# biotite-dev/springcraft

Measured on AMD Instinct MI355X. Metric: ANM modes/sec (Hessian build + full eigensolve), N=2000 C-alpha, higher is better.
Workload: dtype f64; 1 GPU; C3: N=2000 C-alpha ANM, HinsenForceField (no cutoff), full 6000x6000 eigensolve, all modes + vectors; parallelism=independent structures sharded over GPUs, no data-path collective

## Files before the change

### springcraft_amd/csrc/sb2st.hip

```cpp
#include <algorithm>

#include "twostage_internal.h"

namespace {

__global__ void k_xcd_probe(unsigned* mask) {
  unsigned id;
  asm volatile("s_getreg_b32 %0, hwreg(HW_REG_XCC_ID)" : "=s"(id));
  if (threadIdx.x == 0) atomicOr(mask, 1u << (id & 15u));
}
int probe_xcd_count(sc_ctx* ctx, hipStream_t st) {
  SC_TRY(sc_reserve_dc_aux(ctx, 256));
  unsigned* d_mask = reinterpret_cast<unsigned*>(ctx->dc_aux);
  SC_HIP(ctx, hipMemsetAsync(d_mask, 0, sizeof(unsigned), st));
  const int cus = ctx->num_cus > 0 ? ctx->num_cus : 256;
  hipLaunchKernelGGL(k_xcd_probe, dim3((unsigned)(8 * cus)), dim3(64), 0, st, d_mask);
  SC_HIP(ctx, hipGetLastError());
  unsigned h_mask = 0;
  SC_HIP(ctx, hipMemcpyAsync(&h_mask, d_mask, sizeof(unsigned), hipMemcpyDeviceToHost, st));
  SC_HIP(ctx, hipStreamSynchronize(st));
  int count = 0, top = 0;
  for (int b = 0; b < 16; ++b)
    if (h_mask >> b & 1u) { ++count; top = b + 1; }
  ctx->nxcd = (count >= 1 && count == top) ? std::min(count, 8) : 1;
// ... 257 lines not shown
#ifdef CHASE_STAMPS
__device__ unsigned long long g_chase_stamps[16];
#define CHASE_STAMP_DECL unsigned long long cs_prev = 0, cs_n = 0, cs_sum[12] = {0, 0, 0, 0, 0, 0, 0, 0, 0, 0, 0, 0};
#define CHASE_STAMP(i)                                                                 \
  {                                                                                    \
    unsigned long long t_;                                                             \
    asm volatile("s_memtime %0\n\ts_waitcnt lgkmcnt(0)" : "=s"(t_)::"memory");        \
    if ((i) != 0) cs_sum[i] += t_ - cs_prev;                                           \
    cs_prev = t_;                                                                      \
  }
#define CHASE_STAMP_WRITE                                                                          \
  if ((threadIdx.x & 63) == 0) {                                                                   \
    for (int i_ = 1; i_ < 12; ++i_) atomicAdd(&g_chase_stamps[i_], cs_sum[i_]);                    \
    atomicAdd(&g_chase_stamps[15], cs_n);                                                          \
  }
#else
#define CHASE_STAMP_DECL
#define CHASE_STAMP(i)
#define CHASE_STAMP_WRITE
#endif
template <int SPREAD>
__global__ __launch_bounds__(256, 2) void k_bulge_chase(double* __restrict__ sb_all, SbLayout SL, int batch, int W, int nxcd,
                                                     int* __restrict__ progress, int* __restrict__ next_sweep,
                                                     int* __restrict__ ctl, int give_up_after, v4i* __restrict__ early) {
  constexpr int LD = kB + 1;
  __shared__ double E[kB * LD];
  double* D = E;
  __shared__ double vbuf[2][kB], u[kB], red[4 * kB];
  __shared__ double s_tau, s_beta, s_beta_in;
  __shared__ int s_go, s_claim, s_mode;

  const int n = SL.n;
  const int tid = threadIdx.x;
  const int i = tid & 63, q = tid >> 6;
  __shared__ int s_xcd, s_slot;
  if (tid == 0) {
    unsigned id;
    asm volatile("s_getreg_b32 %0, hwreg(HW_REG_XCC_ID)" : "=s"(id));
    s_xcd = (int)(id & 7u) % nxcd;
    s_slot = atomicAdd(ctl + 2 + s_xcd, 1);
  }
  __syncthreads();
  const int xcd = s_xcd, slot = s_slot;
  const int mpx = xcd < batch ? (batch - xcd + nxcd - 1) / nxcd : 0;
  if (mpx == 0 || slot >= mpx * W) return;
  const int K0 = chase_len(n, 0);
  int tasks_left = give_up_after;

  CHASE_STAMP_DECL
  int cur = slot % mpx, exhausted = 0;
  while (exhausted < mpx) {
    const int b = xcd + nxcd * cur;
    int* prog = progress + (size_t)b * n;
    if (tid == 0) s_claim = atomicAdd(next_sweep + b, 1);
    __syncthreads();
    const int s = __builtin_amdgcn_readfirstlane(s_claim);
    __syncthreads();
    if (s > n - 3) {
      ++exhausted;
      cur = cur + 1 < mpx ? cur + 1 : 0;
      continue;
    }
    exhausted = 0;
    double* sb = sb_all + (size_t)b * SL.slab;
    double* ab = sb + SL.ab;
    {
      const int len = chase_len(n, s);
      const int S = s / kG, cc = s - S * kG;
      const size_t dia0 = (size_t)S * K0 - (size_t)S * (S - 1) / 2;
      const int len_prev = s > 0 ? chase_len(n, s - 1) : 0;
      double tau_p = 0.0;
      for (int k = 0; k < len; ++k) {
        double* vp = vbuf[(k + 1) & 1];
        double* vn = vbuf[k & 1];
        const bool early_task = early != nullptr && s > 0 && k + 1 < len_prev;
        CHASE_STAMP(0)
        if (tid == 0) {
          const int need = s > 0 ? min(k + (early_task ? 1 : 2), len_prev) : 0;
          const int stop0 = __hip_atomic_load(ctl, __ATOMIC_RELAXED, __HIP_MEMORY_SCOPE_AGENT);
          int have = s > 0 ? __hip_atomic_load(prog + s - 1, __ATOMIC_RELAXED, __HIP_MEMORY_SCOPE_AGENT) : 0;
          int go = stop0 ? 0 : 1;
          int mode = 0;
          double beta_in = 0.0;
          const v4i* rec = early_task ? early + ((size_t)b * n + s - 1) * kEarlyRing + ((k + 1) & (kEarlyRing - 1)) : nullptr;
          long spins = 0;
          while (go) {
            if (have >= need) {
              if (!early_task) break;
              if (have >= k + 2) { mode = 2; break; }
              const v4i r = ld16_l2(rec);
              if (r.z == k + 2) {
                mode = 1;
                beta_in = __longlong_as_double((long long)(((unsigned long long)(unsigned)r.y << 32) | (unsigned)r.x));
                break;
              }
            }
            ++spins;
            if (spins > (1L << 21) ||
                ((spins & 15) == 0 && __hip_atomic_load(ctl, __ATOMIC_RELAXED, __HIP_MEMORY_SCOPE_AGENT))) {
              if (!__hip_atomic_load(ctl, __ATOMIC_RELAXED, __HIP_MEMORY_SCOPE_AGENT)) {
                ctl[10] = b; ctl[11] = s; ctl[12] = k;
              }
              __hip_atomic_store(ctl, 1, __ATOMIC_RELAXED, __HIP_MEMORY_SCOPE_AGENT);
              go = 0;
              break;
            }
            __builtin_amdgcn_s_sleep(1);
            have = __hip_atomic_load(prog + s - 1, __ATOMIC_RELAXED, __HIP_MEMORY_SCOPE_AGENT);
          }
          s_go = go;
          s_mode = mode;
          s_beta_in = beta_in;
        }
        __syncthreads();
        if (!s_go) return;
        CHASE_STAMP(1)
        const int mode = s_mode;
#define CHASE_SECOND_WAIT()                                                                                       \
        if (mode == 1) {                                                                                          \
          if (tid == 0) {                                                                                         \
            int go = 1;                                                                                           \
            long spins = 0;                                                                                       \
            while (__hip_atomic_load(prog + s - 1, __ATOMIC_RELAXED, __HIP_MEMORY_SCOPE_AGENT) < k + 2) {         \
              ++spins;                                                                                            \
              if (spins > (1L << 21) ||                                                                           \
                  ((spins & 15) == 0 && __hip_atomic_load(ctl, __ATOMIC_RELAXED, __HIP_MEMORY_SCOPE_AGENT))) {    \
                if (!__hip_atomic_load(ctl, __ATOMIC_RELAXED, __HIP_MEMORY_SCOPE_AGENT)) {                        \
                  ctl[10] = b; ctl[11] = s; ctl[12] = k;                                                          \
                }                                                                                                 \
                __hip_atomic_store(ctl, 1, __ATOMIC_RELAXED, __HIP_MEMORY_SCOPE_AGENT);                           \
                go = 0;                                                                                           \
                break;                                                                                            \
              }                                                                                                   \
              __builtin_amdgcn_s_sleep(1);                                                                        \
            }                                                                                                     \
            s_go = go;                                                                                            \
          }                                                                                                       \
          __syncthreads();                                                                                        \
          if (!s_go) return;                                                                                      \
        }

        const int r0 = s + 1 + k * kB;
        const int L = min(kB, n - r0);
        const size_t dia = dia0 + k;
        double* vd = sb + SL.vd + dia * kDiaSize + (size_t)cc * kG + cc;
        gdptr colbase_k = wave_uniform(ab + (size_t)r0 * kLdab);
        double d16[16];
#pragma unroll
        for (int c = 0; c < 16; ++c) {
          const int jc = min(q * 16 + c, L - 1);
          const int ic = min(max(i, jc), L - 1);
          d16[c] = ld_l2(colbase_k + (unsigned)((ic - jc) + jc * kLdab));
        }
        if (k > 0) {
          gdptr ebase_k = wave_uniform(ab + (size_t)(r0 - kB) * kLdab);
          double t16[16];
          {
            const int ic = min(i, L - 1);
#pragma unroll
            for (int c = 0; c < 16; ++c) {
              const int jj = q * 16 + c;
              t16[c] = ld_l2(ebase_k + (unsigned)((kB + ic - jj) + jj * kLdab));
            }
#pragma unroll
            for (int c = 0; c < 16; ++c) t16[c] = i < L ? t16[c] : 0.0;
            if (mode == 1 && i == kB - 1) {
              const double bin = s_beta_in;
#pragma unroll
              for (int c = 0; c < 16; ++c) t16[c] = q * 16 + c == kB - 1 ? bin : 0.0;
            }
          }
          {
            double a = 0.0;
#pragma unroll
            for (int c = 0; c < 16; ++c) a += t16[c] * vp[q * 16 + c];
            red[q * kB + i] = a;
          }
          lds_barrier();
          CHASE_STAMP(2)
          {
            const double ui = tau_p * ((red[i] + red[kB + i]) + (red[2 * kB + i] + red[3 * kB + i]));
#pragma unroll
            for (int c = 0; c < 16; ++c) {
              t16[c] -= ui * vp[q * 16 + c];
              E[i * LD + q * 16 + c] = t16[c];
            }
          }
          if (q == 0) {
            const double x = t16[0];
            const double t2 = wave_sum((i >= 1 && i < L) ? x * x : 0.0);
            const HH h = householder(__shfl(x, 0), t2);
            vn[i] = i == 0 ? 1.0 : (i < L ? x * h.scale : 0.0);
            if (i == 0) {
              s_tau = h.tau; s_beta = h.beta;
              if (early) {
                const unsigned long long bb = (unsigned long long)__double_as_longlong(h.beta);
                if (SPREAD) st16_sc1(early + ((size_t)b * n + s) * kEarlyRing + (k & (kEarlyRing - 1)), v4i{(int)(unsigned)bb, (int)(unsigned)(bb >> 32), k + 1, 0});
                else st16(early + ((size_t)b * n + s) * kEarlyRing + (k & (kEarlyRing - 1)), v4i{(int)(unsigned)bb, (int)(unsigned)(bb >> 32), k + 1, 0});
              }
            }
          }
          lds_barrier();
          CHASE_STAMP(3)
          {
            double a = 0.0;
#pragma unroll
            for (int ii = q * 16; ii < q * 16 + 16; ++ii) a += E[ii * LD + i] * vn[ii];
            red[q * kB + i] = a;
          }
          lds_barrier();
          if (tid < kB) u[tid] = s_tau * ((red[tid] + red[kB + tid]) + (red[2 * kB + tid] + red[3 * kB + tid]));
          lds_barrier();
          CHASE_STAMP(4)
          CHASE_SECOND_WAIT()
          CHASE_STAMP(5)
#pragma unroll
          for (int c = 0; c < 16; ++c) {
            const int jj = q * 16 + c;
            double e = t16[c] - vn[i] * u[jj];
            if (jj == 0) e = i == 0 ? s_beta : 0.0;
            if (i < L) st_band<SPREAD>(ebase_k + (unsigned)((kB + i - jj) + jj * kLdab), e);
          }
        } else {
          gdptr col_s = wave_uniform(ab + (size_t)s * kLdab);
          if (tid < 64) {
            const double xr = ld_l2(col_s + (unsigned)(1 + min(tid, L - 1)));
            double x = tid < L ? xr : 0.0;
            if (mode == 1 && tid == kB - 1) x = s_beta_in;
            const double t2 = wave_sum(tid >= 1 ? x * x : 0.0);
            const HH h = householder(__shfl(x, 0), t2);
            vn[tid] = tid == 0 ? 1.0 : x * h.scale;
            if (tid == 0) { s_tau = h.tau; s_beta = h.beta; }
          }
          lds_barrier();
          CHASE_STAMP(4)
          CHASE_SECOND_WAIT()
          CHASE_STAMP(5)
          if (tid < L) st_band<SPREAD>(col_s + (unsigned)(1 + tid), tid == 0 ? s_beta : 0.0);
        }
#undef CHASE_SECOND_WAIT
        if (mode == 1 && i == kB - 1) {
#pragma unroll
          for (int c = 0; c < 16; ++c) {
            const int jc = q * 16 + c;
            d16[c] = ld_l2(colbase_k + (unsigned)((kB - 1 - jc) + jc * kLdab));
          }
        }
#pragma unroll
        for (int c = 0; c < 16; ++c) {
          const int jj = q * 16 + c;
          if (i >= jj) {
            const double x = (i < L) ? d16[c] : 0.0;
            D[i * LD + jj] = x;
            D[jj * LD + i] = x;
          }
        }
        lds_barrier();
        CHASE_STAMP(6)
        {
          double a = 0.0;
#pragma unroll
          for (int jj = q * 16; jj < q * 16 + 16; ++jj) a += D[i * LD + jj] * vn[jj];
          red[q * kB + i] = a;
        }
        lds_barrier();
        CHASE_STAMP(7)
        const double tau_now = s_tau;
        if (tid < 64) {
          const double pp = tau_now * ((red[tid] + red[kB + tid]) + (red[2 * kB + tid] + red[3 * kB + tid]));
          const double dot = wave_sum(pp * vn[tid]);
          u[tid] = pp - 0.5 * tau_now * dot * vn[tid];
        }
        lds_barrier();
        CHASE_STAMP(8)
        for (int jj = q * 16; jj < q * 16 + 16; ++jj)
          if (i >= jj && i < L)
            st_band<SPREAD>(colbase_k + (unsigned)((i - jj) + jj * kLdab), D[i * LD + jj] - vn[i] * u[jj] - u[i] * vn[jj]);
        if (tid < L) vd[(size_t)tid * kG] = vn[tid];
        if (tid == 0) sb[SL.tau2 + dia * kG + cc] = tau_now;
        tau_p = tau_now;
        CHASE_STAMP(9)
        asm volatile("s_waitcnt vmcnt(0)" ::: "memory");
        __syncthreads();
        CHASE_STAMP(10)
        if (tid == 0) {
          __hip_atomic_store(prog + s, k + 1, __ATOMIC_RELAXED, __HIP_MEMORY_SCOPE_AGENT);
          if (k + 1 == len) atomicAdd(ctl + 16 + xcd, 1);
          if (give_up_after > 0 && --tasks_left == 0) {
            ctl[1] = give_up_after;
            __hip_atomic_store(ctl, 1, __ATOMIC_RELAXED, __HIP_MEMORY_SCOPE_AGENT);
          }
        }
        CHASE_STAMP(11)
#ifdef CHASE_STAMPS
        ++cs_n;
#endif
      }
    }
  }
  CHASE_STAMP_WRITE
}

constexpr int kSlotE = kB * (kB + 1);
constexpr int kSlotD = 17 * 128;
constexpr int kSlot = kSlotE + kSlotD;
constexpr int kTeamLds = 2 * kB + kB + 4 * kB + 8;
constexpr size_t kPairLdsBytes = sizeof(double) * (3 * kSlot + 2 * kTeamLds);

#ifdef PAIR_STAMPS
__device__ unsigned long long g_pair_stamps[48];
__shared__ unsigned long long s_pair_stamps[48];
#define PAIR_STAMP(var) unsigned long long var; asm volatile("s_memtime %0\n\ts_waitcnt lgkmcnt(0)" : "=s"(var)::"memory");
#define PAIR_ACC(slot, a, b) if (tid == 0) s_pair_stamps[slot] += (b) - (a);
#define PAIR_ACC_B(slot, a, b) if (tid == 256) s_pair_stamps[16 + (slot)] += (b) - (a);
#define PAIR_FLUSH(first)                                                                         \
  for (int i_ = 0; i_ < 16; ++i_)                                                                 \
    if (s_pair_stamps[(first) + i_]) atomicAdd(&g_pair_stamps[(first) + i_], s_pair_stamps[(first) + i_]);
#else
#define PAIR_STAMP(var)
#define PAIR_ACC(slot, a, b)
#define PAIR_ACC_B(slot, a, b)
#define PAIR_FLUSH(first)
#endif

typedef double __attribute__((address_space(3)))* ldptr;
struct PairStepArgs {
  double* ab;
  double* vd;
  double* tau2;
  ldptr slots;
  ldptr vbuf, u, red, sc;
  int* prog;
  int s, k;
  size_t dia;
  int cc;
  int tid;
};

template <int TEAM>
__device__ __forceinline__ void pair_step_full(const PairStepArgs& P, double& tau_p, int& pend_k) {
  const int tid = P.tid, tt = tid & 255, i = tid & 63;
  const int q = (tid >> 6) & 3;
  const int k = P.k, s = P.s;
  const int r0 = s + 1 + k * kB;
  ldptr vp = P.vbuf + ((k + 1) & 1) * kB;
  ldptr vn = P.vbuf + (k & 1) * kB;
  ldptr Eimg = P.slots + (k % 3) * kSlot;
  ldptr Dimg = Eimg + kSlotE;
  ldptr red = P.red;
  ldptr u = P.u;
  gdptr colbase_k = wave_uniform(P.ab + (size_t)r0 * kLdab);
  gdptr ebase_k = wave_uniform(P.ab + (size_t)(r0 - kB) * kLdab);
  const unsigned o_e = (unsigned)(kB + i + q * 16 * (kLdab - 1));
  const unsigned o_d = (unsigned)(i + q * 16 * (kLdab - 1));
  double d16[16], t16[16], vr[16];
  PAIR_STAMP(f0)
  if (TEAM == 0) {
#pragma unroll
    for (int c = 0; c < 16; ++c) t16[c] = ld_l2(ebase_k + (o_e + (unsigned)(c * (kLdab - 1))));
  } else {
    const ldptr En = P.slots + ((k + 1) % 3) * kSlot;
    const int i1 = min(i + 1, kB - 1);
    const ldptr rowD = i < kB - 1 ? Dimg + i1 * (i1 + 1) / 2 : En;
    const ldptr rowE = Eimg + i1 * (kB + 1) + 1;
#pragma unroll
    for (int c = 0; c < 16; ++c) d16[c] = rowD[q * 16 + c + 1];
#pragma unroll
    for (int c = 0; c < 16; ++c) t16[c] = i < kB - 1 ? rowE[q * 16 + c] : 0.0;
    if (q == 3) {
      const double dcol = Dimg[i1 * (i1 + 1) / 2];
      t16[15] = i < kB - 1 ? dcol : En[0];
      if (i == kB - 1) d16[15] = En[kSlotE];
    }
    PAIR_STAMP(g1)
    asm volatile("s_waitcnt vmcnt(0)" ::: "memory");
    PAIR_STAMP(g2)
    PAIR_ACC_B(10, f0, g1) PAIR_ACC_B(11, g1, g2)
  }
#pragma unroll
  for (int c = 0; c < 16; ++c) vr[c] = vp[q * 16 + c];
  PAIR_STAMP(fa)
  lds_barrier();
  PAIR_STAMP(f1)
  PAIR_ACC(12, f0, fa)
  if (TEAM == 1) {
    if (tt == 0 && pend_k >= 0) __hip_atomic_store(P.prog + s, pend_k + 1, __ATOMIC_RELAXED, __HIP_MEMORY_SCOPE_AGENT);
    pend_k = k;
  } else {
#pragma unroll
    for (int c = 0; c < 16; ++c) d16[c] = ld_l2(colbase_k + (o_d + (unsigned)(c * (kLdab - 1))));
  }
  {
    double a = 0.0;
#pragma unroll
    for (int c = 0; c < 16; ++c) a += t16[c] * vr[c];
    red[q * kB + i] = a;
  }
  lds_barrier();
  {
    const double ui = tau_p * ((red[i] + red[kB + i]) + (red[2 * kB + i] + red[3 * kB + i]));
    ldptr erow = Eimg + i * (kB + 1) + q * 16;
#pragma unroll
    for (int c = 0; c < 16; ++c) {
      t16[c] -= ui * vr[c];
      erow[c] = t16[c];
    }
    if (q == 0) {
      const double x = t16[0];
      const double t2 = wave_sum(i >= 1 ? x * x : 0.0);
      const HH h = householder(__shfl(x, 0), t2);
      vn[i] = i == 0 ? 1.0 : x * h.scale;
      if (i == 0) { P.sc[0] = h.tau; P.sc[1] = h.beta; }
    }
  }
  lds_barrier();
  PAIR_STAMP(f3)
#pragma unroll
  for (int c = 0; c < 16; ++c) vr[c] = vn[q * 16 + c];
  {
    double a = 0.0;
    const ldptr ecol = Eimg + q * 16 * (kB + 1) + i;
#pragma unroll
    for (int c = 0; c < 16; ++c) a += ecol[c * (kB + 1)] * vr[c];
    red[q * kB + i] = a;
  }
  lds_barrier();
  if (tt < kB) u[tt] = P.sc[0] * ((red[tt] + red[kB + tt]) + (red[2 * kB + tt] + red[3 * kB + tt]));
  {
    ldptr rowp = Dimg + i * (i + 1) / 2 + q * 16;
#pragma unroll
    for (int c = 0; c < 16; ++c) {
      d16[c] = q * 16 + c <= i ? d16[c] : 0.0;
      if (q * 16 + c <= i) rowp[c] = d16[c];
    }
  }
  lds_barrier();
  PAIR_STAMP(f5)
  {
    const double vi = vn[i];
#pragma unroll
    for (int c = 0; c < 16; ++c) t16[c] -= vi * u[q * 16 + c];
    if (q == 0) t16[0] = i == 0 ? P.sc[1] : 0.0;
    if (TEAM == 0) {
      ldptr erow = Eimg + i * (kB + 1) + q * 16;
#pragma unroll
      for (int c = 0; c < 16; ++c) erow[c] = t16[c];
      if (q == 0 && i >= 1) ebase_k[(unsigned)(kB + i)] = 0.0;
    } else {
#pragma unroll
      for (int c = 0; c < 16; ++c) ebase_k[o_e + (unsigned)(c * (kLdab - 1))] = t16[c];
    }
    double a = 0.0;
#pragma unroll
    for (int c = 0; c < 16; ++c) {
      const int ii = q * 16 + c;
      const double dcolv = Dimg[ii * (ii + 1) / 2 + min(i, ii)];
      a += (d16[c] + (ii > i ? dcolv : 0.0)) * vr[c];
    }
    red[q * kB + i] = a;
  }
  lds_barrier();
  PAIR_STAMP(f6)
  const double tau_f = P.sc[0];
  if (tt < kB) {
    const double pp = tau_f * ((red[tt] + red[kB + tt]) + (red[2 * kB + tt] + red[3 * kB + tt]));
    const double dot = wave_sum(pp * vn[tt]);
    u[tt] = pp - 0.5 * tau_f * dot * vn[tt];
  }
  lds_barrier();
  PAIR_STAMP(f7)
  {
    const double vi = vn[i], wi = u[i];
    if (TEAM == 0) {
      ldptr rowp = Dimg + i * (i + 1) / 2 + q * 16;
#pragma unroll
      for (int c = 0; c < 16; ++c)
        if (q * 16 + c <= i) rowp[c] = d16[c] - vi * u[q * 16 + c] - wi * vr[c];
    } else {
#pragma unroll
      for (int c = 0; c < 16; ++c)
        if (q * 16 + c <= i) colbase_k[o_d + (unsigned)(c * (kLdab - 1))] = d16[c] - vi * u[q * 16 + c] - wi * vr[c];
    }
    double* vd = P.vd + P.dia * kDiaSize + (size_t)P.cc * kG + P.cc;
    if (tt < kB) vd[(size_t)tt * kG] = vn[tt];
    if (tt == 0) P.tau2[P.dia * kG + P.cc] = tau_f;
    tau_p = tau_f;
  }
#ifdef PAIR_STAMPS
  {
    PAIR_STAMP(f8)
    PAIR_ACC(1, f0, f1) PAIR_ACC(2, f1, f3) PAIR_ACC(3, f3, f5) PAIR_ACC(4, f5, f6) PAIR_ACC(5, f6, f7) PAIR_ACC(6, f7, f8)
    PAIR_ACC_B(1, f0, f1) PAIR_ACC_B(2, f1, f3) PAIR_ACC_B(3, f3, f5) PAIR_ACC_B(4, f5, f6) PAIR_ACC_B(5, f6, f7)
    PAIR_ACC_B(13, f7, f8)
  }
#endif
}

struct PairGenArgs {
  double* ab;
  double* vd;
  double* tau2;
  ldptr slots;
  ldptr vbuf, u, red, sc;
  int* prog;
  int* sweeps_done;
  int n, s, k, my_len, team, to_lds;
  size_t dia0;
  int cc, tid;
};
struct PairCarry {
  double tau_p;
  int pend_k;
};

__device__ __noinline__ PairCarry pair_step_general(const PairGenArgs P, double tau_p, int pend_k) {
  double* const ab = P.ab;
  const ldptr slots = P.slots, vbuf = P.vbuf, u = P.u, red = P.red, sc = P.sc;
  int* const prog = P.prog;
  const int n = P.n, s = P.s, k = P.k, my_len = P.my_len, team = P.team, cc = P.cc, tid = P.tid;
  const bool to_lds = P.to_lds != 0;
  const size_t dia0 = P.dia0;
  const int tt = tid & 255, i = tid & 63, q = (tid >> 6) & 3;
  const bool active = k >= 0 && k < my_len;
  const bool first = k == 0;
  const bool eph = active && !first;
  const int kk = active ? k : 0;
  const int r0 = s + 1 + kk * kB;
  const int L = active ? min(kB, n - r0) : 0;
  ldptr vp = vbuf + ((kk + 1) & 1) * kB;
  ldptr vn = vbuf + (kk & 1) * kB;
  ldptr Eimg = slots + (kk % 3) * kSlot;
  ldptr Dimg = Eimg + kSlotE;
  const size_t dia = dia0 + kk;
  gdptr colbase_k = wave_uniform(ab + (size_t)r0 * kLdab);
  gdptr ebase_k = wave_uniform(ab + (size_t)(r0 - (first ? 0 : kB)) * kLdab);

  double d16[16], t16[16];
  double xcol = 0.0;
#pragma unroll
  for (int c = 0; c < 16; ++c) { d16[c] = 0.0; t16[c] = 0.0; }
  if (active && team == 0) {
    if (!first) {
      const int ic = min(i, L - 1);
#pragma unroll
      for (int c = 0; c < 16; ++c) {
        const int jj = q * 16 + c;
        t16[c] = ld_l2(ebase_k + (unsigned)((kB + ic - jj) + jj * kLdab));
      }
    } else if (q == 0) {
      gdptr col_s = wave_uniform(ab + (size_t)s * kLdab);
      xcol = ld_l2(col_s + (unsigned)(1 + min(i, L - 1)));
    }
#pragma unroll
    for (int c = 0; c < 16; ++c) {
      const int jc = min(q * 16 + c, L - 1);
      const int ic = min(max(i, jc), L - 1);
      d16[c] = ld_l2(colbase_k + (unsigned)((ic - jc) + jc * kLdab));
    }
  } else if (active) {
    const ldptr En = slots + ((kk + 1) % 3) * kSlot;
    const int i1 = min(i + 1, kB - 1);
    const ldptr rowD = i < kB - 1 ? Dimg + i1 * (i1 + 1) / 2 : En;
    const ldptr rowE = Eimg + i1 * (kB + 1) + 1;
#pragma unroll
    for (int c = 0; c < 16; ++c) d16[c] = rowD[q * 16 + c + 1];
    if (!first) {
#pragma unroll
      for (int c = 0; c < 16; ++c) t16[c] = i < kB - 1 ? rowE[q * 16 + c] : 0.0;
    }
    if (q == 3) {
      const double dcol = Dimg[i1 * (i1 + 1) / 2];
      if (!first) t16[15] = i < kB - 1 ? dcol : En[0];
      if (i == kB - 1) d16[15] = En[kSlotE];
    }
    if (first && q == 0) xcol = i < kB - 1 ? Dimg[i1 * (i1 + 1) / 2] : En[0];
  }
#pragma unroll
  for (int c = 0; c < 16; ++c) t16[c] = i < L ? t16[c] : 0.0;
  xcol = i < L ? xcol : 0.0;
  if (!to_lds || !active) asm volatile("s_waitcnt vmcnt(0)" ::: "memory");
  lds_barrier();
  if (tt == 0 && pend_k >= 0) {
    __hip_atomic_store(prog + s, pend_k + 1, __ATOMIC_RELAXED, __HIP_MEMORY_SCOPE_AGENT);
    if (pend_k + 1 == my_len) atomicAdd(P.sweeps_done, 1);
  }
  pend_k = -1;

  if (eph) {
    double a = 0.0;
#pragma unroll
    for (int c = 0; c < 16; ++c) a += t16[c] * vp[q * 16 + c];
    red[q * kB + i] = a;
  }
  lds_barrier();
  if (eph) {
    const double ui = tau_p * ((red[i] + red[kB + i]) + (red[2 * kB + i] + red[3 * kB + i]));
#pragma unroll
    for (int c = 0; c < 16; ++c) {
      t16[c] -= ui * vp[q * 16 + c];
      Eimg[i * (kB + 1) + q * 16 + c] = t16[c];
    }
    if (q == 0) xcol = t16[0];
  }
  if (active && q == 0) {
    const double t2 = wave_sum((i >= 1 && i < L) ? xcol * xcol : 0.0);
    const HH h = householder(__shfl(xcol, 0), t2);
    vn[i] = i == 0 ? 1.0 : (i < L ? xcol * h.scale : 0.0);
    if (i == 0) { sc[0] = h.tau; sc[1] = h.beta; }
    if (first && i < L) {
      gdptr col_s = wave_uniform(ab + (size_t)s * kLdab);
      col_s[(unsigned)(1 + i)] = i == 0 ? h.beta : 0.0;
    }
  }
  lds_barrier();
  if (eph) {
    double a = 0.0;
#pragma unroll
    for (int ii = q * 16; ii < q * 16 + 16; ++ii) a += Eimg[ii * (kB + 1) + i] * vn[ii];
    red[q * kB + i] = a;
  }
  lds_barrier();
  if (eph && tt < kB) u[tt] = sc[0] * ((red[tt] + red[kB + tt]) + (red[2 * kB + tt] + red[3 * kB + tt]));
#pragma unroll
  for (int c = 0; c < 16; ++c) d16[c] = (i < L && q * 16 + c <= i) ? d16[c] : 0.0;
  if (active) {
    ldptr rowp = Dimg + i * (i + 1) / 2 + q * 16;
#pragma unroll
    for (int c = 0; c < 16; ++c)
      if (q * 16 + c <= i) rowp[c] = d16[c];
  }
  lds_barrier();
  if (eph) {
    const double vi = vn[i], beta = sc[1];
#pragma unroll
    for (int c = 0; c < 16; ++c) {
      const int jj = q * 16 + c;
      double e = t16[c] - vi * u[jj];
      if (jj == 0) e = i == 0 ? beta : 0.0;
      if (to_lds) {
        Eimg[i * (kB + 1) + jj] = i < L ? e : 0.0;
        if (jj == 0 && i >= 1 && i < L) ebase_k[(unsigned)(kB + i)] = 0.0;
      } else if (i < L) {
        ebase_k[(unsigned)((kB + i - jj) + jj * kLdab)] = e;
      }
    }
  }
  if (active) {
    double a = 0.0;
#pragma unroll
    for (int c = 0; c < 16; ++c) a += d16[c] * vn[q * 16 + c];
#pragma unroll
    for (int ii = q * 16; ii < q * 16 + 16; ++ii) {
      const double dv = Dimg[ii * (ii + 1) / 2 + min(i, ii)];
      a += ii > i ? dv * vn[ii] : 0.0;
    }
    red[q * kB + i] = a;
  }
  lds_barrier();
    const double tau_now = sc[0];
  if (active && tt < kB) {
    const double pp = tau_now * ((red[tt] + red[kB + tt]) + (red[2 * kB + tt] + red[3 * kB + tt]));
    const double dot = wave_sum(pp * vn[tt]);
    u[tt] = pp - 0.5 * tau_now * dot * vn[tt];
  }
  lds_barrier();
  if (active) {
    const double vi = vn[i], wi = u[i];
#pragma unroll
    for (int c = 0; c < 16; ++c) {
      const int jj = q * 16 + c;
      if (jj <= i) {
        const double val = d16[c] - vi * u[jj] - wi * vn[jj];
        if (to_lds) {
          Dimg[i * (i + 1) / 2 + jj] = i < L ? val : 0.0;
          if (first && i == 0) colbase_k[0] = val;
        } else if (i < L) {
          colbase_k[(unsigned)((i - jj) + jj * kLdab)] = val;
        }
      }
    }
    double* vd = P.vd + dia * kDiaSize + (size_t)cc * kG + cc;
    if (tt < L) vd[(size_t)tt * kG] = vn[tt];
    if (tt == 0) P.tau2[dia * kG + cc] = tau_now;
    tau_p = tau_now;
    if (!to_lds) pend_k = k;
  }
  return PairCarry{tau_p, pend_k};
}

struct PairLayout {
  int n;
  long long slab, ab, vd, tau2;
};

__device__ __forceinline__ bool pair_common_step(bool hasB, int m, int lenA, int sA, int n) {
  return hasB && m >= 3 && m < lenA && sA + 1 + (m + 1) * kB <= n;
}

__global__ __launch_bounds__(512, 1) void k_bulge_pair(double* __restrict__ sb_all, PairLayout SL, int batch, int W, int nxcd,
                                                       int* __restrict__ progress, int* __restrict__ next_pair,
                                                       int* __restrict__ ctl, int give_up_after) {
  extern __shared__ __attribute__((aligned(16))) double pair_lds[];
  __shared__ int s_go, s_claim, s_xcd, s_slot;

  const int n = SL.n;
  const int tid = threadIdx.x;
  const int wave = __builtin_amdgcn_readfirstlane(tid >> 6);
  const int team = wave >> 2;
  const int tt = tid & 255;
  double* const slots = pair_lds;
  double* const tl = pair_lds + 3 * kSlot + team * kTeamLds;
  double* const vbuf = tl;
  double* const u = tl + 2 * kB;
  double* const red = tl + 3 * kB;
  double* const sc = tl + 7 * kB;

  if (tid == 0) {
    unsigned id;
    asm volatile("s_getreg_b32 %0, hwreg(HW_REG_XCC_ID)" : "=s"(id));
    s_xcd = (int)(id & 7u) % nxcd;
    s_slot = atomicAdd(ctl + 2 + s_xcd, 1);
  }
#ifdef PAIR_STAMPS
  if (tid < 48) s_pair_stamps[tid] = 0;
#endif
  __syncthreads();
  const int xcd = s_xcd, slot = s_slot;
  const int mpx = xcd < batch ? (batch - xcd + nxcd - 1) / nxcd : 0;
  if (mpx == 0 || slot >= mpx * W) return;
  const int K0 = chase_len(n, 0);
  int steps_left = give_up_after;

  int cur = slot % mpx, exhausted = 0;
  while (exhausted < mpx) {
    const int b = xcd + nxcd * cur;
    int* prog = progress + (size_t)b * n;
    if (tid == 0) s_claim = atomicAdd(next_pair + b, 1);
    __syncthreads();
    const int sA = 2 * __builtin_amdgcn_readfirstlane(s_claim);
    __syncthreads();
    if (sA > n - 3) {
      ++exhausted;
      cur = cur + 1 < mpx ? cur + 1 : 0;
      continue;
    }
    exhausted = 0;
    double* sb = sb_all + (size_t)b * SL.slab;
    double* ab = sb + SL.ab;
    const bool hasB = sA + 1 <= n - 3;
    const int lenA = chase_len(n, sA), lenB = hasB ? chase_len(n, sA + 1) : 0;
    const int s = sA + team;
    const int my_len = team ? lenB : lenA;
    const int S = s / kG, cc = s - S * kG;
    const size_t dia0 = (size_t)S * K0 - (size_t)S * (S - 1) / 2;
    const int len_prev = sA > 0 ? chase_len(n, sA - 1) : 0;
    const bool to_lds = team == 0 && hasB;
    double tau_p = 0.0;

    const int nsteps = hasB ? lenA + 2 : lenA;
    int have_c = 0;
    int pend_k = -1;
    for (int m = 0; m < nsteps; ++m) {
      PAIR_STAMP(ts0)
      if (tid == 256) {
        const int need = (sA > 0 && m < lenA) ? min(m + 2, len_prev) : 0;
        int go = 1;
        if (have_c < need || (m & 7) == 0) {
#ifdef PAIR_STAMPS
          s_pair_stamps[16 + 14] += 1ull;
#endif
          const int want = need;
          const int stop0 = __hip_atomic_load(ctl, __ATOMIC_RELAXED, __HIP_MEMORY_SCOPE_AGENT);
          int have = sA > 0 ? __hip_atomic_load(prog + sA - 1, __ATOMIC_RELAXED, __HIP_MEMORY_SCOPE_AGENT) : 0;
          if (stop0) go = 0;
          long spins = 0;
          while (go && have < want) {
            ++spins;
            if (spins > (1L << 21) ||
                ((spins & 15) == 0 && __hip_atomic_load(ctl, __ATOMIC_RELAXED, __HIP_MEMORY_SCOPE_AGENT))) {
              if (!__hip_atomic_load(ctl, __ATOMIC_RELAXED, __HIP_MEMORY_SCOPE_AGENT)) {
                ctl[10] = b; ctl[11] = sA; ctl[12] = m;
              }
              __hip_atomic_store(ctl, 1, __ATOMIC_RELAXED, __HIP_MEMORY_SCOPE_AGENT);
              go = 0;
              break;
            }
            __builtin_amdgcn_s_sleep(1);
            have = __hip_atomic_load(prog + sA - 1, __ATOMIC_RELAXED, __HIP_MEMORY_SCOPE_AGENT);
          }
          have_c = have;
        }
        s_go = go;
      }
      PAIR_STAMP(tsp)
      lds_barrier();
      if (!s_go) {
        asm volatile("s_waitcnt vmcnt(0)" ::: "memory");
        __syncthreads();
        if (tt == 0 && pend_k >= 0) __hip_atomic_store(prog + s, pend_k + 1, __ATOMIC_RELAXED, __HIP_MEMORY_SCOPE_AGENT);
        if (hasB) {
          for (int pos = max(m - 2, 0); pos < min(m, lenA); ++pos) {
            const double* Es = slots + (pos % 3) * kSlot;
            const double* Ds = Es + kSlotE;
            const int r0p = sA + 1 + pos * kB;
            const int Lp = min(kB, n - r0p);
            const int i_lo = (pos == m - 2 && pos >= 1) ? 1 : 0;
            if (pos > 0)
              for (int e = tid; e < kB * kB; e += 512) {
                const int ii = e & 63, jj = e >> 6;
                if (ii >= i_lo && ii < Lp) ab[(size_t)(r0p - kB + jj) * kLdab + (kB + ii - jj)] = Es[ii * (kB + 1) + jj];
              }
            for (int e = tid; e < kB * kB; e += 512) {
              const int ii = e & 63, jj = e >> 6;
              if (ii >= jj && ii >= i_lo && ii < Lp) ab[(size_t)(r0p + jj) * kLdab + (ii - jj)] = Ds[ii * (ii + 1) / 2 + jj];
            }
          }
          asm volatile("s_waitcnt vmcnt(0)" ::: "memory");
          __syncthreads();
          if (tid == 0) {
            __hip_atomic_store(prog + sA, min(m, lenA), __ATOMIC_RELAXED, __HIP_MEMORY_SCOPE_AGENT);
            __hip_atomic_store(prog + sA + 1, min(max(m - 2, 0), lenB), __ATOMIC_RELAXED, __HIP_MEMORY_SCOPE_AGENT);
          }
        }
        if (tid == 0) { PAIR_FLUSH(0) }
        if (tid == 256) { PAIR_FLUSH(16) }
        return;
      }

      PAIR_STAMP(ts1)
      const int k = team ? m - 2 : m;
      if (pair_common_step(hasB, m, lenA, sA, n)) {
        PairStepArgs pa{ab, sb + SL.vd, sb + SL.tau2, (ldptr)slots, (ldptr)vbuf, (ldptr)u, (ldptr)red, (ldptr)sc, prog, s, k,
                        dia0 + k, cc, tid};
        if (team == 0) pair_step_full<0>(pa, tau_p, pend_k);
        else pair_step_full<1>(pa, tau_p, pend_k);
#ifdef PAIR_STAMPS
        if (tid == 0) { s_pair_stamps[9] += 1ull; s_pair_stamps[0] += ts1 - ts0; }
        if (tid == 256) { s_pair_stamps[16] += ts1 - ts0; s_pair_stamps[16 + 7] += tsp - ts0; }
#endif
      } else {
        PairGenArgs ga{ab, sb + SL.vd, sb + SL.tau2, (ldptr)slots, (ldptr)vbuf, (ldptr)u, (ldptr)red, (ldptr)sc, prog,
                       ctl + 16 + xcd, n, s, k, my_len, team, to_lds ? 1 : 0, dia0, cc, tid};
        const PairCarry pc = pair_step_general(ga, tau_p, pend_k);
        tau_p = pc.tau_p;
        pend_k = pc.pend_k;
      }
#ifdef PAIR_STAMPS
      if (tid == 0) s_pair_stamps[8] += 1ull;
#endif
      if (tid == 0) {
        if (to_lds && m + 1 == lenA) atomicAdd(ctl + 16 + xcd, 1);
        if (give_up_after > 0 && --steps_left == 0) {
          ctl[1] = give_up_after;
          __hip_atomic_store(ctl, 1, __ATOMIC_RELAXED, __HIP_MEMORY_SCOPE_AGENT);
        }
      }
    }
    asm volatile("s_waitcnt vmcnt(0)" ::: "memory");
    __syncthreads();
    if (tt == 0 && pend_k >= 0) {
      __hip_atomic_store(prog + s, pend_k + 1, __ATOMIC_RELAXED, __HIP_MEMORY_SCOPE_AGENT);
      if (pend_k + 1 == my_len) atomicAdd(ctl + 16 + xcd, 1);
    }
    if (tid == 0 && hasB) __hip_atomic_store(prog + sA, lenA, __ATOMIC_RELAXED, __HIP_MEMORY_SCOPE_AGENT);
  }
  if (tid == 0) { PAIR_FLUSH(0) }
  if (tid == 256) { PAIR_FLUSH(16) }
}

}


static int launch_chase(sc_ctx* ctx, sc_host::ChaseForm form, int n, int batch, double* d_sb_ws, const SbLayout& SL,
                        SbTimers& timers, bool* chased) {
  using sc_host::ChaseForm;
  hipStream_t st = ctx->stream;
  const bool pair = form == ChaseForm::Pair;
  int per_cu = 0;
  const hipError_t oe =
      pair ? hipOccupancyMaxActiveBlocksPerMultiprocessor(&per_cu, k_bulge_pair, 512, kPairLdsBytes)
           : (form == ChaseForm::Spread ? hipOccupancyMaxActiveBlocksPerMultiprocessor(&per_cu, k_bulge_chase<1>, 256, 0)
                                        : hipOccupancyMaxActiveBlocksPerMultiprocessor(&per_cu, k_bulge_chase<0>, 256, 0));
  if (oe != hipSuccess) per_cu = 0;
  const sc_host::ChaseLaunch L =
      sc_host::chase_launch(sc_host::two_stage_env(), form, n, batch, ctx->nxcd, ctx->num_cus, per_cu);
  if (L.W < 1) return SC_OK;
  SC_TRY(sc_reserve_dc_aux(ctx, L.prog_bytes + L.next_bytes + L.early_bytes));
  int* d_prog = reinterpret_cast<int*>(ctx->dc_aux);
  int* d_next = reinterpret_cast<int*>(reinterpret_cast<char*>(ctx->dc_aux) + L.prog_bytes);
  int* d_ctl = ctx->d_chase_ctl;
  v4i* d_early = L.early_bytes ? reinterpret_cast<v4i*>(reinterpret_cast<char*>(ctx->dc_aux) + L.prog_bytes + L.next_bytes)
                               : nullptr;
  SC_HIP(ctx, hipMemsetAsync(ctx->dc_aux, 0, L.prog_bytes + L.next_bytes + L.early_bytes, st));
  SC_HIP(ctx, hipMemsetAsync(d_ctl, 0, kChaseCtlInts * sizeof(int), st));
  timers.bulge.start();
  if (pair)
    hipLaunchKernelGGL(k_bulge_pair, dim3((unsigned)L.grid), dim3(512), kPairLdsBytes, st, d_sb_ws,
                       PairLayout{SL.n, SL.slab, SL.ab, SL.vd, SL.tau2}, batch, L.W, L.nxcd, d_prog, d_next, d_ctl,
                       ctx->chase_give_up);
  else if (form == ChaseForm::Spread)
    hipLaunchKernelGGL(k_bulge_chase<1>, dim3((unsigned)L.grid), dim3(256), 0, st, d_sb_ws, SL, batch, L.W, L.nxcd, d_prog,
                       d_next, d_ctl, ctx->chase_give_up, d_early);
  else
    hipLaunchKernelGGL(k_bulge_chase<0>, dim3((unsigned)L.grid), dim3(256), 0, st, d_sb_ws, SL, batch, L.W, L.nxcd, d_prog,
                       d_next, d_ctl, ctx->chase_give_up, d_early);
  const hipError_t le = hipGetLastError();
  timers.bulge.stop();
  if (le != hipSuccess) {
    if (pair) {
      ctx->pair_attr = 0;
      ++ctx->cnt_pair_fallbacks;
    }
    return SC_OK;
  }
  hipLaunchKernelGGL(k_chase_finish, dim3((unsigned)batch), dim3(256), 0, st, d_sb_ws, SL, batch, L.nxcd, d_prog,
                     (const int*)d_ctl, ctx->d_status);
  SC_HIP(ctx, hipGetLastError());
  ++ctx->cnt_chase_launches;
  if (pair) ++ctx->cnt_pair_launches;
  ctx->last_chase_ctl = d_ctl;
  ctx->chase_ctl_xcds = L.nxcd;
  *chased = true;
  return SC_OK;
}

static int chase_stepwise(sc_ctx* ctx, int n, int batch, double* d_sb_ws, const SbLayout& SL) {
  const sc_host::TwoStageEnv& E = sc_host::two_stage_env();
  hipStream_t st = ctx->stream;
  const int t_max = 2 * (n - 3) + chase_len(n, n - 3) - 1;
  const int gx = chase_len(n, 0) / 2 + 1;
  const int nparts = sc_host::bulge_stream_parts(E, batch);
  if (nparts > 1) {
    SC_TRY(sc_aux_stream(ctx));
    SC_TRY(sc_side_streams(ctx, nparts - 1));
    SC_HIP(ctx, hipEventRecord(ctx->aux_fork, st));
    for (int p = 1; p < nparts; ++p) SC_HIP(ctx, hipStreamWaitEvent(ctx->side_streams[p - 1], ctx->aux_fork, 0));
    const int burst = sc_host::bulge_burst(E);
    for (int t0 = 0; t0 <= t_max; t0 += burst)
      for (int p = 0; p < nparts; ++p) {
        const int lo = (int)((long long)batch * p / nparts), hi = (int)((long long)batch * (p + 1) / nparts);
        for (int t = t0; t <= std::min(t_max, t0 + burst - 1); ++t)
          hipLaunchKernelGGL(k_bulge_step, dim3((unsigned)gx, (unsigned)(hi - lo)), dim3(256), 0,
                             p == 0 ? st : ctx->side_streams[p - 1], d_sb_ws + (size_t)lo * SL.slab, SL, t);
      }
    for (int p = 1; p < nparts; ++p) {
      SC_HIP(ctx, hipEventRecord(ctx->side_joins[p - 1], ctx->side_streams[p - 1]));
      SC_HIP(ctx, hipStreamWaitEvent(st, ctx->side_joins[p - 1], 0));
    }
  } else {
    for (int t = 0; t <= t_max; ++t)
      hipLaunchKernelGGL(k_bulge_step, dim3((unsigned)gx, (unsigned)batch), dim3(256), 0, st, d_sb_ws, SL, t);
  }
  return SC_OK;
}

int sb_stage2(sc_ctx* ctx, double* d_a, long long stride_a, int n, int batch, double* d_tri_ws, const TriLayout& TL,
              double* d_sb_ws, const SbLayout& SL, double* d_band_copy, SbTimers& timers) {
  hipStream_t st = ctx->stream;
  hipLaunchKernelGGL(k_band_extract, dim3(256, (unsigned)batch), dim3(256), 0, st, d_a, stride_a, d_sb_ws, SL);
  if (d_band_copy)
    SC_HIP(ctx, hipMemcpyAsync(d_band_copy, d_sb_ws + SL.ab, sizeof(double) * kLdab * n, hipMemcpyDeviceToDevice, st));
  hipLaunchKernelGGL(k_sb_clean, dim3((unsigned)n, (unsigned)batch), dim3(256), 0, st, d_a, stride_a, n);
  for (int b = 0; b < batch; ++b) {
    double* sb = d_sb_ws + (size_t)b * SL.slab;
    SC_HIP(ctx, hipMemsetAsync(sb + SL.vd, 0, sizeof(double) * (size_t)SL.ndia * kDiaSize, st));
    SC_HIP(ctx, hipMemsetAsync(sb + SL.tau2, 0, sizeof(double) * (size_t)SL.ndia * kG, st));
  }
// ... 56 lines not shown
```

Before: 182,000 modes/s.

## Fuse band-chase pair step phases with DPP wave reductions to cut LDS barriers

Reworks the bulge-chasing pair step in the symmetric band-to-tridiagonal reduction so that each wave computes the Householder reflector redundantly, using DPP-based wave sums and readfirstlane instead of LDS round-trips. The E-block column sums become a register transpose-reduce, and the dot product for the symmetric update is folded into the preceding reduction. Together these remove several LDS barriers and intermediate LDS writes per chase step. The cost is extra cross-lane DPP instructions and more register pressure, and the summation order changes slightly.

```diff
diff --git a/springcraft_amd/csrc/sb2st.hip b/springcraft_amd/csrc/sb2st.hip
--- a/springcraft_amd/csrc/sb2st.hip
+++ b/springcraft_amd/csrc/sb2st.hip
@@ -583,6 +583,7 @@
 }
 
 constexpr int kSlotE = kB * (kB + 1);
+constexpr int kSlotDUsed = kB * (kB + 1) / 2;
 constexpr int kSlotD = 17 * 128;
 constexpr int kSlot = kSlotE + kSlotD;
 constexpr int kTeamLds = 2 * kB + kB + 4 * kB + 8;
@@ -592,6 +593,8 @@
 __device__ unsigned long long g_pair_stamps[48];
 __shared__ unsigned long long s_pair_stamps[48];
 #define PAIR_STAMP(var) unsigned long long var; asm volatile("s_memtime %0\n\ts_waitcnt lgkmcnt(0)" : "=s"(var)::"memory");
+#define PAIR_STAMP_VAR(var) unsigned long long var = 0;
+#define PAIR_STAMP_SET(var) asm volatile("s_memtime %0\n\ts_waitcnt lgkmcnt(0)" : "=s"(var)::"memory");
 #define PAIR_ACC(slot, a, b) if (tid == 0) s_pair_stamps[slot] += (b) - (a);
 #define PAIR_ACC_B(slot, a, b) if (tid == 256) s_pair_stamps[16 + (slot)] += (b) - (a);
 #define PAIR_FLUSH(first)                                                                         \
@@ -599,12 +602,94 @@
     if (s_pair_stamps[(first) + i_]) atomicAdd(&g_pair_stamps[(first) + i_], s_pair_stamps[(first) + i_]);
 #else
 #define PAIR_STAMP(var)
+#define PAIR_STAMP_VAR(var)
+#define PAIR_STAMP_SET(var)
 #define PAIR_ACC(slot, a, b)
 #define PAIR_ACC_B(slot, a, b)
 #define PAIR_FLUSH(first)
 #endif
 
+template <int CTRL>
+__device__ __forceinline__ double pair_dpp(double x) {
+  const unsigned long long b = (unsigned long long)__double_as_longlong(x);
+  const int lo = __builtin_amdgcn_update_dpp(0, (int)(unsigned)b, CTRL, 0xf, 0xf, true);
+  const int hi = __builtin_amdgcn_update_dpp(0, (int)(unsigned)(b >> 32), CTRL, 0xf, 0xf, true);
+  return __longlong_as_double((long long)(((unsigned long long)(unsigned)hi << 32) | (unsigned long long)(unsigned)lo));
+}
+template <int CTRL, int ROWS>
+__device__ __forceinline__ double pair_dpp_bcast(double x) {
+  const unsigned long long b = (unsigned long long)__double_as_longlong(x);
+  const int lo = __builtin_amdgcn_update_dpp(0, (int)(unsigned)b, CTRL, ROWS, 0xf, false);
+  const int hi = __builtin_amdgcn_update_dpp(0, (int)(unsigned)(b >> 32), CTRL, ROWS, 0xf, false);
+  return __longlong_as_double((long long)(((unsigned long long)(unsigned)hi << 32) | (unsigned long long)(unsigned)lo));
+}
+__device__ __forceinline__ double pair_sum63(double x) {
+  x += pair_dpp<0x111>(x);
+  x += pair_dpp<0x112>(x);
+  x += pair_dpp<0x114>(x);
+  x += pair_dpp<0x118>(x);
+  x += pair_dpp_bcast<0x142, 0xa>(x);
+  x += pair_dpp_bcast<0x143, 0xc>(x);
+  return x;
+}
+__device__ __forceinline__ double pair_sum_all(double x) {
+  const unsigned long long b = (unsigned long long)__double_as_longlong(pair_sum63(x));
+  const unsigned lo = (unsigned)__builtin_amdgcn_readlane((int)(unsigned)b, 63);
+  const unsigned hi = (unsigned)__builtin_amdgcn_readlane((int)(unsigned)(b >> 32), 63);
+  return __longlong_as_double((long long)(((unsigned long long)hi << 32) | (unsigned long long)lo));
+}
+__device__ __forceinline__ int pair_sum16_index(int lane) {
+  return 8 * (lane & 1) + 4 * ((lane >> 1) & 1) + 2 * ((lane >> 2) & 1) + ((lane >> 3) & 1);
+}
+__device__ __forceinline__ double pair_sum16(const double (&v)[16], int lane) {
+  const bool b0 = (lane & 1) != 0, b1 = (lane & 2) != 0, b2 = (lane & 4) != 0, b3 = (lane & 8) != 0;
+  double k8[8], k4[4], k2[2];
+#pragma unroll
+  for (int k = 0; k < 8; ++k) {
+    const double send = b0 ? v[k] : v[k + 8];
+    k8[k] = (b0 ? v[k + 8] : v[k]) + pair_dpp<0xB1>(send);
+  }
+#pragma unroll
+  for (int k = 0; k < 4; ++k) {
+    const double send = b1 ? k8[k] : k8[k + 4];
+    k4[k] = (b1 ? k8[k + 4] : k8[k]) + pair_dpp<0x4E>(send);
+  }
+#pragma unroll
+  for (int k = 0; k < 2; ++k) {
+    const double send = b2 ? k4[k] : k4[k + 2];
+    const double from_lo = pair_dpp<0x114>(send), from_hi = pair_dpp<0x104>(send);
+    k2[k] = (b2 ? k4[k + 2] : k4[k]) + (b2 ? from_lo : from_hi);
+  }
+  double r = (b3 ? k2[1] : k2[0]) + pair_dpp<0x128>(b3 ? k2[0] : k2[1]);
+  r += __shfl_xor(r, 16);
+  r += __shfl_xor(r, 32);
+  return r;
+}
 typedef double __attribute__((address_space(3)))* ldptr;
+struct PairRefl {
+  double vi, tau, beta;
+};
+__device__ __forceinline__ PairRefl pair_reflector(double x, int lane) {
+  const double t2 = pair_sum_all(lane >= 1 ? x * x : 0.0);
+  const unsigned long long b = (unsigned long long)__double_as_longlong(x);
+  const unsigned lo = (unsigned)__builtin_amdgcn_readfirstlane((int)(unsigned)b);
+  const unsigned hi = (unsigned)__builtin_amdgcn_readfirstlane((int)(unsigned)(b >> 32));
+  const HH h = householder(__longlong_as_double((long long)(((unsigned long long)hi << 32) | (unsigned long long)lo)), t2);
+  return PairRefl{lane == 0 ? 1.0 : x * h.scale, h.tau, h.beta};
+}
+__device__ __forceinline__ void pair_colsums(const double (&e16)[16], double vi, double tau, int lane, ldptr uq) {
+  double x[16];
+#pragma unroll
+  for (int c = 0; c < 16; ++c) x[c] = e16[c] * vi;
+  const double r = pair_sum16(x, lane);
+  if (lane < 16) uq[pair_sum16_index(lane)] = tau * r;
+}
+__device__ __forceinline__ double pair_w(ldptr red, ldptr dots, double tau, double vi, int lane) {
+  const double pp = tau * ((red[lane] + red[kB + lane]) + (red[2 * kB + lane] + red[3 * kB + lane]));
+  const double dot = tau * ((dots[0] + dots[1]) + (dots[2] + dots[3]));
+  return fma(-(0.5 * tau * dot), vi, pp);
+}
+
 struct PairStepArgs {
   double* ab;
   double* vd;
@@ -628,6 +713,7 @@
   ldptr vn = P.vbuf + (k & 1) * kB;
   ldptr Eimg = P.slots + (k % 3) * kSlot;
   ldptr Dimg = Eimg + kSlotE;
+  ldptr col0 = Dimg + kSlotDUsed;
   ldptr red = P.red;
   ldptr u = P.u;
   gdptr colbase_k = wave_uniform(P.ab + (size_t)r0 * kLdab);
@@ -676,38 +762,37 @@
 #pragma unroll
     for (int c = 0; c < 16; ++c) a += t16[c] * vr[c];
     red[q * kB + i] = a;
+    if (q == 0) col0[i] = t16[0];
   }
   lds_barrier();
+  double vi, tau_f;
+  PAIR_STAMP_VAR(f3) PAIR_STAMP_VAR(f7)
   {
     const double ui = tau_p * ((red[i] + red[kB + i]) + (red[2 * kB + i] + red[3 * kB + i]));
-    ldptr erow = Eimg + i * (kB + 1) + q * 16;
-#pragma unroll
-    for (int c = 0; c < 16; ++c) {
-      t16[c] -= ui * vr[c];
-      erow[c] = t16[c];
-    }
-    if (q == 0) {
-      const double x = t16[0];
-      const double t2 = wave_sum(i >= 1 ? x * x : 0.0);
-      const HH h = householder(__shfl(x, 0), t2);
-      vn[i] = i == 0 ? 1.0 : x * h.scale;
-      if (i == 0) { P.sc[0] = h.tau; P.sc[1] = h.beta; }
-    }
-  }
-  lds_barrier();
-  PAIR_STAMP(f3)
-#pragma unroll
-  for (int c = 0; c < 16; ++c) vr[c] = vn[q * 16 + c];
-  {
-    double a = 0.0;
-    const ldptr ecol = Eimg + q * 16 * (kB + 1) + i;
-#pragma unroll
-    for (int c = 0; c < 16; ++c) a += ecol[c * (kB + 1)] * vr[c];
-    red[q * kB + i] = a;
-  }
-  lds_barrier();
-  if (tt < kB) u[tt] = P.sc[0] * ((red[tt] + red[kB + tt]) + (red[2 * kB + tt] + red[3 * kB + tt]));
-  {
+    const double x = fma(-ui, vp[0], col0[i]);
+#pragma unroll
+    for (int c = 0; c < 16; ++c) t16[c] = fma(-ui, vr[c], t16[c]);
+    if (q == 0) t16[0] = x;
+    const PairRefl h = pair_reflector(x, i);
+    vi = h.vi;
+    tau_f = h.tau;
+    if ((i >> 4) == q) vn[i] = vi;
+    PAIR_STAMP_SET(f3)
+    pair_colsums(t16, vi, tau_f, i, u + q * 16);
+#pragma unroll
+    for (int c = 0; c < 16; ++c) vr[c] = vn[q * 16 + c];
+#pragma unroll
+    for (int c = 0; c < 16; ++c) t16[c] -= vi * u[q * 16 + c];
+    if (q == 0) t16[0] = i == 0 ? h.beta : 0.0;
+    if (TEAM == 0) {
+      ldptr erow = Eimg + i * (kB + 1) + q * 16;
+#pragma unroll
+      for (int c = 0; c < 16; ++c) erow[c] = t16[c];
+      if (q == 0 && i >= 1) ebase_k[(unsigned)(kB + i)] = 0.0;
+    } else {
+#pragma unroll
+      for (int c = 0; c < 16; ++c) ebase_k[o_e + (unsigned)(c * (kLdab - 1))] = t16[c];
+    }
     ldptr rowp = Dimg + i * (i + 1) / 2 + q * 16;
 #pragma unroll
     for (int c = 0; c < 16; ++c) {
@@ -715,22 +800,10 @@
       if (q * 16 + c <= i) rowp[c] = d16[c];
     }
   }
+  PAIR_STAMP(f4)
   lds_barrier();
   PAIR_STAMP(f5)
   {
-    const double vi = vn[i];
-#pragma unroll
-    for (int c = 0; c < 16; ++c) t16[c] -= vi * u[q * 16 + c];
-    if (q == 0) t16[0] = i == 0 ? P.sc[1] : 0.0;
-    if (TEAM == 0) {
-      ldptr erow = Eimg + i * (kB + 1) + q * 16;
-#pragma unroll
-      for (int c = 0; c < 16; ++c) erow[c] = t16[c];
-      if (q == 0 && i >= 1) ebase_k[(unsigned)(kB + i)] = 0.0;
-    } else {
-#pragma unroll
-      for (int c = 0; c < 16; ++c) ebase_k[o_e + (unsigned)(c * (kLdab - 1))] = t16[c];
-    }
     double a = 0.0;
 #pragma unroll
     for (int c = 0; c < 16; ++c) {
@@ -739,19 +812,15 @@
       a += (d16[c] + (ii > i ? dcolv : 0.0)) * vr[c];
     }
     red[q * kB + i] = a;
+    const double dq = pair_sum63(vi * a);
+    if (i == kB - 1) P.sc[4 + q] = dq;
   }
   lds_barrier();
   PAIR_STAMP(f6)
-  const double tau_f = P.sc[0];
-  if (tt < kB) {
-    const double pp = tau_f * ((red[tt] + red[kB + tt]) + (red[2 * kB + tt] + red[3 * kB + tt]));
-    const double dot = wave_sum(pp * vn[tt]);
-    u[tt] = pp - 0.5 * tau_f * dot * vn[tt];
-  }
-  lds_barrier();
-  PAIR_STAMP(f7)
   {
-    const double vi = vn[i], wi = u[i];
+    const double wi = pair_w(red, P.sc + 4, tau_f, vi, i);
+    if ((i >> 4) == q) u[i] = wi;
+    PAIR_STAMP_SET(f7)
     if (TEAM == 0) {
       ldptr rowp = Dimg + i * (i + 1) / 2 + q * 16;
 #pragma unroll
@@ -763,7 +832,7 @@
         if (q * 16 + c <= i) colbase_k[o_d + (unsigned)(c * (kLdab - 1))] = d16[c] - vi * u[q * 16 + c] - wi * vr[c];
     }
     double* vd = P.vd + P.dia * kDiaSize + (size_t)P.cc * kG + P.cc;
-    if (tt < kB) vd[(size_t)tt * kG] = vn[tt];
+    if (tt < kB) vd[(size_t)tt * kG] = vi;
     if (tt == 0) P.tau2[P.dia * kG + P.cc] = tau_f;
     tau_p = tau_f;
   }
@@ -771,8 +840,9 @@
   {
     PAIR_STAMP(f8)
     PAIR_ACC(1, f0, f1) PAIR_ACC(2, f1, f3) PAIR_ACC(3, f3, f5) PAIR_ACC(4, f5, f6) PAIR_ACC(5, f6, f7) PAIR_ACC(6, f7, f8)
+    PAIR_ACC(15, f4, f5)
     PAIR_ACC_B(1, f0, f1) PAIR_ACC_B(2, f1, f3) PAIR_ACC_B(3, f3, f5) PAIR_ACC_B(4, f5, f6) PAIR_ACC_B(5, f6, f7)
-    PAIR_ACC_B(13, f7, f8)
+    PAIR_ACC_B(13, f7, f8) PAIR_ACC_B(15, f4, f5)
   }
 #endif
 }
@@ -877,16 +947,12 @@
   if (eph) {
     const double ui = tau_p * ((red[i] + red[kB + i]) + (red[2 * kB + i] + red[3 * kB + i]));
 #pragma unroll
-    for (int c = 0; c < 16; ++c) {
-      t16[c] -= ui * vp[q * 16 + c];
-      Eimg[i * (kB + 1) + q * 16 + c] = t16[c];
-    }
+    for (int c = 0; c < 16; ++c) t16[c] = fma(-ui, vp[q * 16 + c], t16[c]);
     if (q == 0) xcol = t16[0];
   }
   if (active && q == 0) {
-    const double t2 = wave_sum((i >= 1 && i < L) ? xcol * xcol : 0.0);
-    const HH h = householder(__shfl(xcol, 0), t2);
-    vn[i] = i == 0 ? 1.0 : (i < L ? xcol * h.scale : 0.0);
+    const PairRefl h = pair_reflector(xcol, i);
+    vn[i] = i < L ? h.vi : 0.0;
     if (i == 0) { sc[0] = h.tau; sc[1] = h.beta; }
     if (first && i < L) {
       gdptr col_s = wave_uniform(ab + (size_t)s * kLdab);
@@ -894,14 +960,8 @@
     }
   }
   lds_barrier();
-  if (eph) {
-    double a = 0.0;
-#pragma unroll
-    for (int ii = q * 16; ii < q * 16 + 16; ++ii) a += Eimg[ii * (kB + 1) + i] * vn[ii];
-    red[q * kB + i] = a;
-  }
+  if (eph) pair_colsums(t16, vn[i], sc[0], i, u + q * 16);
   lds_barrier();
-  if (eph && tt < kB) u[tt] = sc[0] * ((red[tt] + red[kB + tt]) + (red[2 * kB + tt] + red[3 * kB + tt]));
 #pragma unroll
   for (int c = 0; c < 16; ++c) d16[c] = (i < L && q * 16 + c <= i) ? d16[c] : 0.0;
   if (active) {
@@ -936,14 +996,12 @@
       a += ii > i ? dv * vn[ii] : 0.0;
     }
     red[q * kB + i] = a;
+    const double dq = pair_sum63(vn[i] * a);
+    if (i == kB - 1) sc[4 + q] = dq;
   }
   lds_barrier();
     const double tau_now = sc[0];
-  if (active && tt < kB) {
-    const double pp = tau_now * ((red[tt] + red[kB + tt]) + (red[2 * kB + tt] + red[3 * kB + tt]));
-    const double dot = wave_sum(pp * vn[tt]);
-    u[tt] = pp - 0.5 * tau_now * dot * vn[tt];
-  }
+  if (active && tt < kB) u[tt] = pair_w(red, sc + 4, tau_now, vn[tt], tt);
   lds_barrier();
   if (active) {
     const double vi = vn[i], wi = u[i];
```

Result: no change. 183,700 modes/s (median of 6 runs) (+0.9%).
